# PRBonn/OverlapNet

Measured on NVIDIA H100. Metric: scan-pairs/sec (overlap+yaw) at 64x900, higher is better.
Workload: dtype f16

## Files before the change

overlapnet_b200/csrc/api.cu:

```cuda
#include "common.cuh"
#include <math.h>
#include <string.h>
#include <algorithm>

using namespace ovn;

static const char* kLegNames[] = {"s_conv1", "s_conv2", "s_conv3", "s_conv3a", "s_conv4", "s_conv5",
                                  "s_conv6", "s_conv7", "s_conv8", "s_conv9", "s_conv10"};

static void set_spec(ConvSpec& L, const char* name, int kh, int kw, int sh, int sw, int cin, int cout, int relu,
                     int h_in, int w_in) {
  memset(&L, 0, sizeof(L));
  snprintf(L.name, sizeof(L.name), "%s", name);
  L.kh = kh; L.kw = kw; L.sh = sh; L.sw = sw; L.cin = cin; L.cout = cout; L.relu = relu;
  L.h_in = h_in; L.w_in = w_in;
  L.h_out = (h_in - kh) / sh + 1;
  L.w_out = (w_in - kw) / sw + 1;
}

static void slot_sizes(const ovn_handle* h, int slot, int64_t* n_kernel, int64_t* n_bias) {
  if (slot == kMaxLegLayers + 3) {
    *n_kernel = h->dense_in; *n_bias = 1;
    return;
  }
// ... 71 lines not shown
    case kErrNonFiniteOperand:
      OVN_SET_ERR(h, OVN_ERR_INVALID_ARG, "a value is not finite in the fp16 operands of the tensor-core path: a feature "
                  "volume given to the heads (NaN, inf, or |x - centre| > 65504; outputs of the call are poisoned, NaN / "
                  "INT32_MIN), or in the tensor-core leg an input pixel (NaN, inf) or an activation of s_conv1 .. the "
                  "last layer but one (above 65504; the feature volumes of the call are not valid)");
    case kErrPeerWait: OVN_SET_ERR(h, OVN_ERR_CUDA, "ovn_peer_wait timed out: a peer rank never signalled");
    case kErrInjectedFault: OVN_SET_ERR(h, OVN_ERR_CUDA, "tensor-core pipeline failed: k_conv2_wgmma: fault injected by "
                                        "OVN_DEBUG_FAULT (code %d); outputs of the call are poisoned (NaN / INT32_MIN)", e);
    case kErrDeltaLeftProducer: case kErrDeltaLeftConsumer: ring = "k_delta_conv1_wgmma: LEFT volume ring"; break;
    case kErrDeltaRightProducer: case kErrDeltaRightConsumer: ring = "k_delta_conv1_wgmma: RIGHT window ring"; break;
    case kErrDeltaW1Producer: case kErrDeltaW1Consumer: ring = "k_delta_conv1_wgmma: W1 ring"; break;
    case kErrDeltaO1Producer: case kErrDeltaO1Consumer: ring = "k_delta_conv1_wgmma: o1 staging"; break;
    case kErrConv2Producer: case kErrConv2Consumer: ring = "k_conv2_wgmma: o1 + W2 ring"; break;
    case kErrConv3X3Producer: case kErrConv3X3Consumer: ring = "k_conv3_wgmma: x3 ring"; break;
    case kErrConv3W3Producer: case kErrConv3W3Consumer: ring = "k_conv3_wgmma: W3 ring"; break;
    case kErrCorrRightProducer: case kErrCorrRightConsumer: ring = "k_corr_wgmma: RIGHT third ring"; break;
    case kErrCorrLeftProducer: case kErrCorrLeftConsumer: ring = "k_corr_wgmma: LEFT tile ring"; break;
  }
  if (!ring) OVN_SET_ERR(h, OVN_ERR_CUDA, "unknown device error code %d", e);
  OVN_SET_ERR(h, OVN_ERR_CUDA, "tensor-core pipeline failed: %s, %s wait timed out (code %d); outputs of the call are "
              "poisoned (NaN / INT32_MIN)", ring, e < 200 ? "producer" : "consumer", e);
}

}

extern "C" {

int ovn_abi_version(void) { return OVN_ABI_VERSION; }

const char* ovn_status_string(int status) {
  switch (status) {
    case OVN_OK: return "OVN_OK";
// ... 1659 lines not shown
```

overlapnet_b200/csrc/common.cuh:

```cuda
#pragma once
#include <cuda_runtime.h>
#include <cuda_fp16.h>
#include <stddef.h>
#include <stdint.h>
#include <stdio.h>
#include <memory>
#include <string>
#include <vector>
#include <map>

#include "../../include/ovn_b200.h"

struct ovn_handle;

namespace ovn {

template <class T, bool Pinned = false>
class Buffer {
 public:
  Buffer() = default;
  Buffer(Buffer&& o) noexcept { swap(o); }
  Buffer& operator=(Buffer&& o) noexcept {
    Buffer old(std::move(o));
    swap(old);
// ... 280 lines not shown
  bool switched = false;
  explicit DeviceGuard(const ovn_handle* h) {
    if (h && cudaGetDevice(&prev) == cudaSuccess && prev != h->device) switched = cudaSetDevice(h->device) == cudaSuccess;
  }
  ~DeviceGuard() { if (switched) cudaSetDevice(prev); }
};

enum DeviceError : int {
  kErrDeltaLeftProducer = 101, kErrDeltaLeftConsumer = 402,
  kErrDeltaRightProducer = 103, kErrDeltaRightConsumer = 404,
  kErrDeltaW1Producer = 102, kErrDeltaW1Consumer = 202,
  kErrDeltaO1Producer = 104, kErrDeltaO1Consumer = 405,
  kErrConv2Producer = 111, kErrConv2Consumer = 211,
  kErrConv3X3Producer = 121, kErrConv3X3Consumer = 221,
  kErrConv3W3Producer = 122, kErrConv3W3Consumer = 222,
  kErrCorrRightProducer = 131, kErrCorrRightConsumer = 231,
  kErrCorrLeftProducer = 132, kErrCorrLeftConsumer = 232,
  kErrInjectedFault = 501,
  kErrBadIndex = 900,
  kErrRowNotPrepared = 901,
  kErrIcpBadIndex = 902,
  kErrNonFiniteOperand = 910,
  kErrPeerWait = 950,
};

inline void prof_mark(ovn_handle* h, int kind, cudaStream_t s) {
  if (!h->profiling) return;
  cudaEvent_t e;
  if (cudaEventCreate(&e) != cudaSuccess) return;
  cudaEventRecord(e, s);
  h->prof_ev[kind].push_back(e);
}
// ... 125 lines not shown
```

overlapnet_b200/csrc/network_tc.cu:

```cuda
#include "common.cuh"
#include "hopper.cuh"

#include <cuda_fp16.h>
#include <stddef.h>
#include <stdlib.h>

namespace ovn {

using namespace hopper;

constexpr int WF = 360;
constexpr int CF = 128;
constexpr int S15 = 15;
constexpr int NB = 24;
constexpr int PAIR_ROWS = NB * NB;
constexpr int K4_PITCH = CF;

struct TcState {
  Buffer<__half> w1p;
  Buffer<__half> w2p;
  Buffer<__half> w3p;
  Buffer<float> b2eff;
  Buffer<__half> wres[kMaxLegLayers];
  Buffer<__half> actp[2];
  Buffer<float> leg_part;
  Buffer<__half> l16;
  Buffer<__half> r16;
  Buffer<__half> o1;
  Buffer<__half> x3;
  Buffer<float> partial;
  Buffer<__half> lc;
  Buffer<__half> rc;
  Buffer<float> corr_part;
  const float* pb_key = nullptr;
  int64_t pb_rows = 0;
  Buffer<__half> pb_l16;
  Buffer<__half> pb_lc;
  Buffer<int32_t> pb_bad;
  Buffer<float> mu;
  bool mu_set = false;
  Buffer<float> mu_o1;
  Buffer<float> mu_x3;
  Buffer<float> b2base;
  Buffer<float> b3eff;
  bool act_set = false;
  int64_t rows_pad = 0;
  int64_t last_n = 0;
};

void TcStateDelete::operator()(TcState* t) const { delete t; }

__host__ __device__ __forceinline__ int k4_pos(int r, int c) {
// ... 60 lines not shown
struct LegArgs {
  const __half* A; int64_t a_pitch;
  int runs_per_img, in_img_planes, in_run_planes;
  int kh, kw, c8in;
  const __half* Bp;
  const float* bias; int n_valid;
  int64_t M;
  __half* out_planes; int64_t out_pitch; int out_run_planes;
  float* out_f32;
  int n_split; float* part;
  int* err;
};

__device__ __forceinline__ bool leg_act_unstorable(float v) { return !(v < 65520.f) || v == -INFINITY; }

constexpr int C6_LROWS = 64, C6_RROWS = 128;
constexpr int C6_LT = 6, C6_RT = 3;
constexpr int C6_L_BYTES = 2 * 16 * C6_LROWS * 16;
constexpr int C6_R_BYTES = 2 * 16 * C6_RROWS * 16;
constexpr int C6_VOL_L_BYTES = C6_LT * C6_L_BYTES;
constexpr int C6_VOL_R_BYTES = C6_RT * C6_R_BYTES;

template <int TR, int NT>
__global__ void __launch_bounds__(256)
k_pack_corr(const float* __restrict__ bank, const int32_t* __restrict__ idx, int n, __half* __restrict__ out,
            int* __restrict__ err, int32_t* __restrict__ row_bad) {
  const int64_t i = (int64_t)blockIdx.x * blockDim.x + threadIdx.x;
  const int64_t per = 16 * NT * TR;
  if (i >= (int64_t)n * per) return;
  const int p = (int)(i / per);
  int r = (int)(i % per);
  const int vrow = r % (NT * TR); r /= NT * TR;
  const int pl = r;
  const int tile = vrow / TR, row = vrow % TR;
  float v[8];
  if (vrow < WF) {
    const int64_t src = (idx ? idx[p] : p);
    const float4 a = __ldg(reinterpret_cast<const float4*>(bank + (src * WF + vrow) * CF + pl * 8));
    const float4 b = __ldg(reinterpret_cast<const float4*>(bank + (src * WF + vrow) * CF + pl * 8 + 4));
    v[0] = a.x; v[1] = a.y; v[2] = a.z; v[3] = a.w; v[4] = b.x; v[5] = b.y; v[6] = b.z; v[7] = b.w;
  } else {
#pragma unroll
    for (int e = 0; e < 8; ++e) v[e] = 0.f;
  }
  __half hi[8], lo[8];
#pragma unroll
  for (int e = 0; e < 8; ++e) {
    hi[e] = __float2half_rn(v[e]);
    lo[e] = __float2half_rn(v[e] - __half2float(hi[e]));
  }
  bool bad = false;
#pragma unroll
  for (int e = 0; e < 8; e += 2) bad |= h2_nonfinite(__halves2half2(hi[e], hi[e + 1]));
  if (bad) {
    if (row_bad) row_bad[p] = 1;
    else atomicCAS(err, 0, kErrNonFiniteOperand);
  }
  __half* base = out + ((size_t)p * NT + tile) * (2 * 16 * TR * 8);
  *reinterpret_cast<uint4*>(base + ((size_t)pl * TR + row) * 8) = *reinterpret_cast<const uint4*>(hi);
  *reinterpret_cast<uint4*>(base + ((size_t)(16 + pl) * TR + row) * 8) = *reinterpret_cast<const uint4*>(lo);
}

constexpr int MMA_THREADS = 128;
constexpr int MMA_ROWS = 64;

__device__ __forceinline__ void mma16816(float (&d)[4], uint32_t a0, uint32_t a1, uint32_t a2, uint32_t a3,
                                         uint32_t b0, uint32_t b1) {
  asm volatile("mma.sync.aligned.m16n8k16.row.col.f32.f16.f16.f32 {%0,%1,%2,%3}, {%4,%5,%6,%7}, {%8,%9}, {%0,%1,%2,%3};"
               : "+f"(d[0]), "+f"(d[1]), "+f"(d[2]), "+f"(d[3])
               : "r"(a0), "r"(a1), "r"(a2), "r"(a3), "r"(b0), "r"(b1));
}

__device__ __forceinline__ uint32_t ld_h2(const __half* p) { return __ldg(reinterpret_cast<const unsigned int*>(p)); }

__device__ __forceinline__ uint32_t absdiff_h2(uint32_t a, uint32_t b) {
// ... 437 lines not shown
          for (int j = 0; j < 16; ++j) {
            const int n = j * 8 + 2 * t;
            sum = fmaf(fmaxf(acc[sub][4 * j + 2 * h] + __ldg(bias + nh * 128 + n), 0.f), __ldg(wrow + n), sum);
            sum = fmaf(fmaxf(acc[sub][4 * j + 2 * h + 1] + __ldg(bias + nh * 128 + n + 1), 0.f), __ldg(wrow + n + 1), sum);
          }
          sum += __shfl_xor_sync(0xffffffffu, sum, 1);
          sum += __shfl_xor_sync(0xffffffffu, sum, 2);
          if (t == 0 && r < M) partial[r * 2 + nh] = valid ? sum : 0.f;
        }
    }
  }
done:
  return;
}

constexpr int C6_PARTS = C6_LT * C6_RT;
constexpr int C6_WG = 2;
constexpr int C6_THREADS = C6_WG * 128 + 32;
constexpr int C6_RING = 3;
constexpr int C6_GPITCH = 132;

struct C6Smem {
  __half R[C6_R_BYTES / 2];
  __half L[C6_RING][C6_L_BYTES / 2];
  float G[C6_WG][C6_LROWS * C6_GPITCH];
  MbarRing<C6_RING> left;
  MbarRing<1> right;
};
static_assert(sizeof(C6Smem) <= 232448, "k_corr_wgmma shared memory");
static_assert(offsetof(C6Smem, L) % 16 == 0, "bulk-copy alignment");

__global__ void __launch_bounds__(C6_THREADS, 1)
k_corr_wgmma(const __half* __restrict__ Lc, const int32_t* __restrict__ l_idx, const __half* __restrict__ Rc,
             int r_per_pair, int n_pairs, float* __restrict__ corr_part, int* __restrict__ err) {
  extern __shared__ __align__(128) uint8_t smem_raw[];
  C6Smem& S = *reinterpret_cast<C6Smem*>(smem_raw);
  const int tid = threadIdx.x, warp = tid >> 5, lane = tid & 31;
  const int q = blockIdx.x % C6_RT;
  const Share share = work_share((int64_t)n_pairs * C6_LT, blockIdx.x / C6_RT, gridDim.x / C6_RT);
  const int u_begin = (int)share.begin, u_end = (int)share.end;
  if (tid == 0) {
    S.left.init(4);
    S.right.init(C6_WG * 4);
    mbar_fence_init();
  }
  __syncthreads();

  if (warp == C6_WG * 4) {
    if (lane == 0) {
      uint32_t ri = 0, ui = 0;
      int key = -1;
      for (int u = u_begin; u < u_end; ++u, ++ui) {
        const int p = u / C6_LT, a = u - p * C6_LT;
        if ((r_per_pair ? p : 0) != key) {
          key = r_per_pair ? p : 0;
          PIPE_WAIT(S.right.acquire(ri, C6_R_BYTES), kErrCorrRightProducer);
          bulk_g2s(S.R, Rc + ((size_t)key * C6_RT + q) * (C6_R_BYTES / 2), C6_R_BYTES, S.right.bar(ri));
          ++ri;
        }
        PIPE_WAIT(S.left.acquire(ui, C6_L_BYTES), kErrCorrLeftProducer);
        bulk_g2s(S.L[S.left.slot(ui)], Lc + ((size_t)(l_idx ? l_idx[p] : p) * C6_LT + a) * (C6_L_BYTES / 2), C6_L_BYTES,
                 S.left.bar(ui));
      }
    }
  } else {
    const int wg = warp >> 2, wi = warp & 3, g = lane >> 2, t = lane & 3, tw = tid & 127;
    float* Gw = S.G[wg];
    const uint32_t r_base = smem_u32(S.R);
    uint32_t ri = 0, ui = 0;
    int key = -1;
    bool failed = false;
    for (int u = u_begin; u < u_end; ++u, ++ui) {
      const int p = u / C6_LT, a = u - p * C6_LT;
      if ((r_per_pair ? p : 0) != key) {
        if (key >= 0) S.right.release(ri - 1);
        key = r_per_pair ? p : 0;
        INFLIGHT_WAIT(S.right.wait(ri), kErrCorrRightConsumer);
        ++ri;
      }
      if ((int)(ui & 1) != wg) continue;
      const uint32_t s = S.left.slot(ui);
      INFLIGHT_WAIT(S.left.wait(ui), kErrCorrLeftConsumer);
      const uint32_t l_base = smem_u32(S.L[s]);
      float acc[64];
#pragma unroll
      for (int e = 0; e < 64; ++e) acc[e] = 0.f;
      wgmma_fence();
#pragma unroll
      for (int c16 = 0; c16 < 8; ++c16) {
        const uint64_t ah = desc_kmajor(l_base + c16 * 2 * C6_LROWS * 16, C6_LROWS * 16, 128, kNoSwizzle);
        const uint64_t al = desc_kmajor(l_base + C6_L_BYTES / 2 + c16 * 2 * C6_LROWS * 16, C6_LROWS * 16, 128, kNoSwizzle);
        const uint64_t bh = desc_kmajor(r_base + c16 * 2 * C6_RROWS * 16, C6_RROWS * 16, 128, kNoSwizzle);
        const uint64_t bl = desc_kmajor(r_base + C6_R_BYTES / 2 + c16 * 2 * C6_RROWS * 16, C6_RROWS * 16, 128, kNoSwizzle);
        wgmma_m64n128k16_ss(acc, ah, bh);
        wgmma_m64n128k16_ss(acc, al, bh);
        wgmma_m64n128k16_ss(acc, ah, bl);
      }
      wgmma_commit();
      wgmma_wait<0>();
      S.left.release(ui);
      named_bar_sync(1 + wg, 128);
#pragma unroll
      for (int j = 0; j < 16; ++j) {
        float* r0 = Gw + (wi * 16 + g) * C6_GPITCH + j * 8 + 2 * t;
        *reinterpret_cast<float2*>(r0) = make_float2(acc[4 * j], acc[4 * j + 1]);
        *reinterpret_cast<float2*>(r0 + 8 * C6_GPITCH) = make_float2(acc[4 * j + 2], acc[4 * j + 3]);
      }
      named_bar_sync(1 + wg, 128);
      const int i_lim = min(C6_LROWS, WF - a * C6_LROWS), j_lim = min(C6_RROWS, WF - q * C6_RROWS);
      float* out = corr_part + ((size_t)p * C6_PARTS + a * C6_RT + q) * WF;
      for (int d = tw; d < WF; d += 128) {
        const int dd = d - (C6_RROWS - 1);
        float sum = 0.f;
        if (d < C6_LROWS + C6_RROWS - 1) {
#pragma unroll 8
          for (int ii = 0; ii < C6_LROWS; ++ii) {
            const int jj = ii - dd;
            if (ii < i_lim && jj >= 0 && jj < j_lim) sum += Gw[ii * C6_GPITCH + jj];
          }
        }
        int k = (a * C6_LROWS - q * C6_RROWS + dd - WF / 2) % WF;
        if (k < 0) k += WF;
        out[k] = sum;
      }
    }
  }
done:
  return;
}

template <int EPI>
__global__ void __launch_bounds__(MMA_THREADS)
k_leg_mma(LegArgs g) {
  const int warp = threadIdx.x >> 5, lane = threadIdx.x & 31, gq = lane >> 2, t = lane & 3;
  const int64_t px0 = (int64_t)blockIdx.y * MMA_ROWS + warp * 16;
  if (px0 >= g.M) return;
  const int nz = (g.n_valid + 63) / 64;
  const int y = blockIdx.x, z = blockIdx.z % nz, slice = blockIdx.z / nz;
  const int64_t in_base = (int64_t)(y / g.runs_per_img) * g.in_img_planes + (int64_t)(y % g.runs_per_img) * g.in_run_planes;
// ... 87 lines not shown
    if (bad) atomicCAS(g.err, 0, kErrNonFiniteOperand);
    __half hi[8], lo[8];
#pragma unroll
    for (int e = 0; e < 8; ++e) {
      hi[e] = __float2half_rn(v[e]);
      lo[e] = __float2half_rn(v[e] - __half2float(hi[e]));
    }
    const int64_t pl = y * g.out_run_planes + c8;
    *reinterpret_cast<uint4*>(g.out_planes + ((size_t)pl * g.out_pitch + px) * 8) = *reinterpret_cast<const uint4*>(hi);
    *reinterpret_cast<uint4*>(g.out_planes + ((size_t)(pl + g.out_run_planes / 2) * g.out_pitch + px) * 8) =
        *reinterpret_cast<const uint4*>(lo);
  } else {
    float* dst = g.out_f32 + (y * g.M + px) * g.n_valid + c8 * 8;
    *reinterpret_cast<float4*>(dst) = make_float4(v[0], v[1], v[2], v[3]);
    *reinterpret_cast<float4*>(dst + 4) = make_float4(v[4], v[5], v[6], v[7]);
  }
}

__global__ void __launch_bounds__(384)
k_corr_finalize(const float* __restrict__ part, float* __restrict__ corr_out, int32_t* __restrict__ yaw,
                const int* __restrict__ err) {
  __shared__ float s_corr[WF];
  const int p = blockIdx.x;
  for (int k = threadIdx.x; k < WF; k += blockDim.x) {
    float c = 0.f;
    for (int b = 0; b < C6_PARTS; ++b) c += part[((size_t)p * C6_PARTS + b) * WF + k];
    s_corr[k] = c;
    if (corr_out) corr_out[(size_t)p * WF + k] = c;
  }
  __syncthreads();
  if (threadIdx.x == 0) {
    int best = 0;
    float bv = s_corr[0];
    for (int k = 1; k < WF; ++k)
      if (s_corr[k] > bv) { bv = s_corr[k]; best = k; }
    yaw[p] = (*err != 0) ? INT32_MIN : 180 - best;
  }
}

__global__ void __launch_bounds__(1024)
k_o1_channel_mean(const __half* __restrict__ o1, int64_t M, float* __restrict__ mu) {
  __shared__ float part[16][64];
  const int o = threadIdx.x & 63, g = threadIdx.x >> 6;
  float acc = 0.f;
  for (int64_t m = g; m < M; m += 16)
    for (int di = 0; di < S15; ++di) acc += __half2float(o1[o1_chunk_offset(m, di, o >> 3) + (o & 7)]);
  part[g][o] = acc;
  __syncthreads();
  if (g == 0) {
    float t = 0.f;
    for (int k = 0; k < 16; ++k) t += part[k][o];
// ... 327 lines not shown
  if ((rc = t->leg_part.ensure(h, part_bytes)) != OVN_OK) return rc;
  for (int b = 0; b < 2; ++b) {
    const size_t bytes = max_planes_bytes * h->cfg.max_batch_scans + 32768;
    if ((rc = t->actp[b].ensure(h, bytes)) != OVN_OK) return rc;
    OVN_CUDA(h, cudaMemset(t->actp[b], 0, bytes));
  }
  const int64_t maxp = h->cfg.max_batch_pairs;
  t->rows_pad = ((maxp * PAIR_ROWS + 1024 + 255) / 256) * 256;
  if ((rc = t->l16.ensure(h, (size_t)maxp * WF * K4_PITCH * sizeof(__half))) != OVN_OK) return rc;
  if ((rc = t->r16.ensure(h, (size_t)maxp * WF * K4_PITCH * sizeof(__half))) != OVN_OK) return rc;
  OVN_CUDA(h, cudaMemset(t->l16, 0, (size_t)maxp * WF * K4_PITCH * sizeof(__half)));
  OVN_CUDA(h, cudaMemset(t->r16, 0, (size_t)maxp * WF * K4_PITCH * sizeof(__half)));
  if ((rc = t->o1.ensure(h, (size_t)120 * t->rows_pad * 8 * sizeof(__half))) != OVN_OK) return rc;
  if ((rc = t->x3.ensure(h, (size_t)16 * t->rows_pad * 8 * sizeof(__half))) != OVN_OK) return rc;
  if ((rc = t->partial.ensure(h, (size_t)t->rows_pad * 2 * sizeof(float))) != OVN_OK) return rc;
  if ((rc = t->lc.ensure(h, (size_t)maxp * C6_VOL_L_BYTES)) != OVN_OK) return rc;
  if ((rc = t->rc.ensure(h, (size_t)maxp * C6_VOL_R_BYTES)) != OVN_OK) return rc;
  if ((rc = t->corr_part.ensure(h, (size_t)maxp * C6_PARTS * WF * sizeof(float))) != OVN_OK) return rc;
  OVN_CUDA(h, cudaFuncSetAttribute(k_delta_conv1_wgmma, cudaFuncAttributeMaxDynamicSharedMemorySize, (int)sizeof(K4Smem)));
  OVN_CUDA(h, cudaFuncSetAttribute(k_conv2_wgmma, cudaFuncAttributeMaxDynamicSharedMemorySize, (int)C2_SMEM));
  OVN_CUDA(h, cudaFuncSetAttribute(k_conv3_wgmma, cudaFuncAttributeMaxDynamicSharedMemorySize, (int)sizeof(C3Smem)));
  OVN_CUDA(h, cudaFuncSetAttribute(k_corr_wgmma, cudaFuncAttributeMaxDynamicSharedMemorySize, (int)sizeof(C6Smem)));
  if ((rc = t->mu.ensure(h, CF * sizeof(float))) != OVN_OK) return rc;
  OVN_CUDA(h, cudaMemset(t->mu, 0, CF * sizeof(float)));
  OVN_CUDA(h, cudaMemset(t->o1, 0, (size_t)120 * t->rows_pad * 8 * sizeof(__half)));
  OVN_CUDA(h, cudaMemset(t->x3, 0, (size_t)16 * t->rows_pad * 8 * sizeof(__half)));
  OVN_CUDA(h, cudaFuncSetAttribute(k_leg_layer1_small<true>, cudaFuncAttributeMaxDynamicSharedMemorySize, (int)L1_SMALL_SMEM));
  OVN_CUDA(h, cudaFuncSetAttribute(k_leg_layer1_small<false>, cudaFuncAttributeMaxDynamicSharedMemorySize, (int)L1_SMALL_SMEM));
  h->tc = std::move(t);
  return OVN_OK;
}

int leg_forward_tc(ovn_handle* h, const float* d_input, int n, float* d_fv, cudaStream_t s, int stop_layer) {
  TcState* t = h->tc.get();
  if (!t) OVN_SET_ERR(h, OVN_ERR_WEIGHTS, "tensor-core weights not packed");
  prof_mark(h, PROF_LEG, s);
  {
// ... 41 lines not shown
      else k_leg_splitk_reduce<4><<<(unsigned)((work + 255) / 256), 256, 0, s>>>(la, n * L.h_out);
    } else if (last) {
      k_leg_mma<3><<<grid, MMA_THREADS, 0, s>>>(la);
    } else {
      k_leg_mma<4><<<grid, MMA_THREADS, 0, s>>>(la);
    }
    OVN_LAUNCH_CHECK(h);
    cur ^= 1;
  }
  prof_mark(h, PROF_LEG, s);
  return OVN_OK;
}

static int calibrate_all(ovn_handle* h, const float* d_vols, const int32_t* d_idx, bool keep_mu, cudaStream_t s);

int tc_bank_release(ovn_handle* h, const float* d_bank) {
  TcState* t = h->tc.get();
  if (!t || (d_bank && t->pb_key != d_bank)) return OVN_OK;
  OVN_CUDA(h, cudaDeviceSynchronize());
  t->pb_l16 = {};
  t->pb_lc = {};
  t->pb_bad = {};
  t->pb_key = nullptr;
  t->pb_rows = 0;
  return OVN_OK;
}

int tc_bank_prepare(ovn_handle* h, const float* d_bank, int64_t capacity, int64_t first, int64_t count, cudaStream_t s) {
  TcState* t = h->tc.get();
  if (!t) OVN_SET_ERR(h, OVN_ERR_WEIGHTS, "tensor-core weights not packed");
  const size_t l16_bytes = (size_t)capacity * WF * K4_PITCH * sizeof(__half);
  if (t->pb_key != d_bank || l16_bytes > t->pb_l16.bytes()) {
    int rc = OVN_OK;
    if (t->pb_key != nullptr || t->pb_l16) rc = tc_bank_release(h, nullptr);
    if (rc == OVN_OK) rc = t->pb_l16.ensure(h, l16_bytes);
    if (rc == OVN_OK) rc = t->pb_lc.ensure(h, (size_t)capacity * C6_VOL_L_BYTES);
    if (rc == OVN_OK) rc = t->pb_bad.ensure(h, (size_t)capacity * sizeof(int32_t));
    if (rc != OVN_OK) return rc;
    OVN_CUDA(h, cudaMemsetAsync(t->pb_l16, 0, l16_bytes, s));
    t->pb_key = d_bank;
    t->pb_rows = 0;
    if (first != 0) OVN_SET_ERR(h, OVN_ERR_INVALID_ARG, "ovn_bank_prepare: a new bank must be prepared from row 0");
  }
  if (first > t->pb_rows) OVN_SET_ERR(h, OVN_ERR_INVALID_ARG, "ovn_bank_prepare: rows [%lld, %lld) were never prepared",
                                      (long long)t->pb_rows, (long long)first);
  const int64_t per = (int64_t)WF * CF / 4, perL = 16 * C6_LT * C6_LROWS;
  const float* src = d_bank + (size_t)first * WF * CF;
  if (!t->mu_set) {
    int rc = calibrate_all(h, src, nullptr, false, s);
    if (rc != OVN_OK) return rc;
  }
  OVN_CUDA(h, cudaMemsetAsync(t->pb_bad + first, 0, (size_t)count * sizeof(int32_t), s));
  k_gather_rows_f16<<<(unsigned)((count * per + 255) / 256), 256, 0, s>>>(src, nullptr, (int)count, t->mu, 0,
                                                                         t->pb_l16 + (size_t)first * WF * K4_PITCH, h->d_err,
                                                                         t->pb_bad + first);
  OVN_LAUNCH_CHECK(h);
  k_pack_corr<C6_LROWS, C6_LT><<<(unsigned)((count * perL + 255) / 256), 256, 0, s>>>(src, nullptr, (int)count,
                                                                      t->pb_lc + (size_t)first * (C6_VOL_L_BYTES / 2), h->d_err,
                                                                      t->pb_bad + first);
  OVN_LAUNCH_CHECK(h);
  if (first + count > t->pb_rows) t->pb_rows = first + count;
  return OVN_OK;
}

static int calibrate_all(ovn_handle* h, const float* d_vols, const int32_t* d_idx, bool keep_mu, cudaStream_t s) {
  TcState* t = h->tc.get();
  const int base = kMaxLegLayers;
  const int64_t per = (int64_t)WF * CF / 4;
  if (!keep_mu) {
    k_channel_mean<<<1, 1024, 0, s>>>(d_vols, d_idx, 1, t->mu);
    OVN_LAUNCH_CHECK(h);
  }
  OVN_CUDA(h, cudaMemsetAsync(t->mu_o1, 0, 64 * sizeof(float), s));
  OVN_CUDA(h, cudaMemsetAsync(t->mu_x3, 0, 128 * sizeof(float), s));
  k_gather_rows_f16<<<(unsigned)((per + 255) / 256), 256, 0, s>>>(d_vols, d_idx, 1, t->mu, 0, t->l16, h->d_err, nullptr);
// ... 67 lines not shown
int heads_forward_tc(ovn_handle* h, const float* d_bank, const float* d_query, const int32_t* d_left,
                     const int32_t* d_right, int n, float* d_overlap, int32_t* d_yaw, float* d_corr,
                     cudaStream_t s) {
  TcState* t = h->tc.get();
  if (!t) OVN_SET_ERR(h, OVN_ERR_WEIGHTS, "tensor-core weights not packed");
  const int maxp = h->cfg.max_batch_pairs;
  const int base = kMaxLegLayers;
  const int64_t per = (int64_t)WF * CF / 4;
  t->last_n = 0;
  if ((!t->mu_set || !t->act_set) && n > 0) {
    int rc = d_query ? calibrate_all(h, d_query, nullptr, t->mu_set, s) : calibrate_all(h, d_bank, d_right, t->mu_set, s);
    if (rc != OVN_OK) return rc;
  }
  const bool resident = (t->pb_key == d_bank) && t->pb_rows > 0;
  const __half* l16 = resident ? t->pb_l16 : t->l16;
  const __half* lc = resident ? t->pb_lc : t->lc;
  int32_t* lidx = nullptr;
  if (resident) {
    lidx = h->d_idx_san + 2 * (size_t)maxp;
    int rc = sanitize_indices(h, d_left, n, t->pb_rows, kErrRowNotPrepared, lidx, s, t->pb_bad);
    if (rc != OVN_OK) return rc;
  } else {
    k_gather_rows_f16<<<(unsigned)((n * per + 255) / 256), 256, 0, s>>>(d_bank, d_left, n, t->mu, 0, t->l16, h->d_err, nullptr);
    OVN_LAUNCH_CHECK(h);
  }
  if (d_query)
    k_gather_rows_f16<<<(unsigned)((per + 255) / 256), 256, 0, s>>>(d_query, nullptr, 1, t->mu, 0, t->r16, h->d_err, nullptr);
  else
    k_gather_rows_f16<<<(unsigned)((n * per + 255) / 256), 256, 0, s>>>(d_bank, d_right, n, t->mu, 0, t->r16, h->d_err, nullptr);
  OVN_LAUNCH_CHECK(h);
  const int64_t M = (int64_t)n * PAIR_ROWS;
// ... 8 lines not shown
  prof_mark(h, PROF_DELTA, s);
  OVN_LAUNCH_CHECK(h);
  const bool inject_fault = getenv("OVN_DEBUG_FAULT") != nullptr;
  prof_mark(h, PROF_CONV2, s);
  k_conv2_wgmma<<<grid2, TC_THREADS, C2_SMEM, s>>>(t->o1, t->w2p, t->b2eff, t->mu_x3, t->x3, t->rows_pad, M,
                                                   inject_fault ? 1 : 0, h->d_err);
  prof_mark(h, PROF_CONV2, s);
  OVN_LAUNCH_CHECK(h);
  prof_mark(h, PROF_CONV3, s);
  k_conv3_wgmma<<<grid3, TC_THREADS, sizeof(C3Smem), s>>>(t->x3, t->rows_pad, t->w3p, t->b3eff, M, h->d_w[base + 3],
                                                          t->partial, h->d_err);
  prof_mark(h, PROF_CONV3, s);
  OVN_LAUNCH_CHECK(h);
  k_dense_finalize<<<n, 256, 0, s>>>(t->partial, h->d_b[base + 3], PAIR_ROWS, d_overlap, h->d_err);
  OVN_LAUNCH_CHECK(h);
  const int64_t perL = 16 * C6_LT * C6_LROWS, perR = 16 * C6_RT * C6_RROWS;
  if (!resident) {
    k_pack_corr<C6_LROWS, C6_LT><<<(unsigned)((n * perL + 255) / 256), 256, 0, s>>>(d_bank, d_left, n, t->lc, h->d_err, nullptr);
    OVN_LAUNCH_CHECK(h);
  }
  if (d_query)
    k_pack_corr<C6_RROWS, C6_RT><<<(unsigned)((perR + 255) / 256), 256, 0, s>>>(d_query, nullptr, 1, t->rc, h->d_err, nullptr);
  else
    k_pack_corr<C6_RROWS, C6_RT><<<(unsigned)((n * perR + 255) / 256), 256, 0, s>>>(d_bank, d_right, n, t->rc, h->d_err, nullptr);
  OVN_LAUNCH_CHECK(h);
  prof_mark(h, PROF_CORR, s);
  const int nc = (int64_t)n * C6_LT < h->sm_count / C6_RT ? n * C6_LT : h->sm_count / C6_RT;
  k_corr_wgmma<<<nc * C6_RT, C6_THREADS, sizeof(C6Smem), s>>>(lc, lidx, t->rc, d_query ? 0 : 1, n, t->corr_part, h->d_err);
  prof_mark(h, PROF_CORR, s);
  OVN_LAUNCH_CHECK(h);
  k_corr_finalize<<<n, 384, 0, s>>>(t->corr_part, d_corr, d_yaw, h->d_err);
  OVN_LAUNCH_CHECK(h);
  t->last_n = n;
  static const bool debug_sync = getenv("OVN_DEBUG_SYNC") != nullptr;
  if (debug_sync) return check_device_error(h, s);
  return OVN_OK;
}

__global__ void __launch_bounds__(256)
k_copy_heads_stage(int stage, const __half* __restrict__ o1, const __half* __restrict__ x3, int64_t x3_pitch,
                   const float* __restrict__ partial, int64_t first, int64_t total, float* __restrict__ out) {
  const int64_t e = (int64_t)blockIdx.x * blockDim.x + threadIdx.x;
  if (e >= total) return;
  out += e;
  if (stage == OVN_STAGE_O1) {
    const int o = (int)(e % 64), jb = (int)(e / 64 % NB), i = (int)(e / (64 * NB) % WF);
// ... 70 lines not shown
```

Before: 212,700.

## Replace tensor-core circular correlation with FP64 FFT spectral correlation for yaw

Swaps the split-fp16 wgmma cross-correlation (pack, corr, finalize) for an FP64 path. A mixed-radix 360-point FFT kernel (radix 8, 9, 5) computes per-channel real spectra of the left and right volumes. A spectral kernel then multiplies and accumulates them across channels, takes an inverse DFT in shared memory, and finds the argmax yaw in the same kernel. This reduces correlation work from O(W^2·C) to O(W log W·C) and removes the partial buffer and finalize launch. In exchange it adds FP64 arithmetic, which has limited throughput on H100, and doubles-sized spectra traffic. Resident banks now cache spectra instead of packed halves.

```diff
diff --git a/overlapnet_b200/csrc/api.cu b/overlapnet_b200/csrc/api.cu
--- a/overlapnet_b200/csrc/api.cu
+++ b/overlapnet_b200/csrc/api.cu
@@ -109,8 +109,8 @@
     case kErrConv2Producer: case kErrConv2Consumer: ring = "k_conv2_wgmma: o1 + W2 ring"; break;
     case kErrConv3X3Producer: case kErrConv3X3Consumer: ring = "k_conv3_wgmma: x3 ring"; break;
     case kErrConv3W3Producer: case kErrConv3W3Consumer: ring = "k_conv3_wgmma: W3 ring"; break;
-    case kErrCorrRightProducer: case kErrCorrRightConsumer: ring = "k_corr_wgmma: RIGHT third ring"; break;
-    case kErrCorrLeftProducer: case kErrCorrLeftConsumer: ring = "k_corr_wgmma: LEFT tile ring"; break;
+    case kErrSpecRightProducer: case kErrSpecRightConsumer: ring = "k_corr_spectral: RIGHT spectrum ring"; break;
+    case kErrSpecLeftProducer: case kErrSpecLeftConsumer: ring = "k_corr_spectral: LEFT spectra ring"; break;
   }
   if (!ring) OVN_SET_ERR(h, OVN_ERR_CUDA, "unknown device error code %d", e);
   OVN_SET_ERR(h, OVN_ERR_CUDA, "tensor-core pipeline failed: %s, %s wait timed out (code %d); outputs of the call are "
diff --git a/overlapnet_b200/csrc/common.cuh b/overlapnet_b200/csrc/common.cuh
--- a/overlapnet_b200/csrc/common.cuh
+++ b/overlapnet_b200/csrc/common.cuh
@@ -318,8 +318,8 @@
   kErrConv2Producer = 111, kErrConv2Consumer = 211,
   kErrConv3X3Producer = 121, kErrConv3X3Consumer = 221,
   kErrConv3W3Producer = 122, kErrConv3W3Consumer = 222,
-  kErrCorrRightProducer = 131, kErrCorrRightConsumer = 231,
-  kErrCorrLeftProducer = 132, kErrCorrLeftConsumer = 232,
+  kErrSpecRightProducer = 133, kErrSpecRightConsumer = 233,
+  kErrSpecLeftProducer = 134, kErrSpecLeftConsumer = 234,
   kErrInjectedFault = 501,
   kErrBadIndex = 900,
   kErrRowNotPrepared = 901,
diff --git a/overlapnet_b200/csrc/network_tc.cu b/overlapnet_b200/csrc/network_tc.cu
--- a/overlapnet_b200/csrc/network_tc.cu
+++ b/overlapnet_b200/csrc/network_tc.cu
@@ -29,13 +29,13 @@
   Buffer<__half> o1;
   Buffer<__half> x3;
   Buffer<float> partial;
-  Buffer<__half> lc;
-  Buffer<__half> rc;
-  Buffer<float> corr_part;
+  Buffer<double2> lspec;
+  Buffer<double2> rspec;
+  Buffer<double2> tw;
   const float* pb_key = nullptr;
   int64_t pb_rows = 0;
   Buffer<__half> pb_l16;
-  Buffer<__half> pb_lc;
+  Buffer<double2> pb_spec;
   Buffer<int32_t> pb_bad;
   Buffer<float> mu;
   bool mu_set = false;
@@ -126,51 +126,97 @@
 
 __device__ __forceinline__ bool leg_act_unstorable(float v) { return !(v < 65520.f) || v == -INFINITY; }
 
-constexpr int C6_LROWS = 64, C6_RROWS = 128;
-constexpr int C6_LT = 6, C6_RT = 3;
-constexpr int C6_L_BYTES = 2 * 16 * C6_LROWS * 16;
-constexpr int C6_R_BYTES = 2 * 16 * C6_RROWS * 16;
-constexpr int C6_VOL_L_BYTES = C6_LT * C6_L_BYTES;
-constexpr int C6_VOL_R_BYTES = C6_RT * C6_R_BYTES;
-
-template <int TR, int NT>
-__global__ void __launch_bounds__(256)
-k_pack_corr(const float* __restrict__ bank, const int32_t* __restrict__ idx, int n, __half* __restrict__ out,
-            int* __restrict__ err, int32_t* __restrict__ row_bad) {
-  const int64_t i = (int64_t)blockIdx.x * blockDim.x + threadIdx.x;
-  const int64_t per = 16 * NT * TR;
-  if (i >= (int64_t)n * per) return;
-  const int p = (int)(i / per);
-  int r = (int)(i % per);
-  const int vrow = r % (NT * TR); r /= NT * TR;
-  const int pl = r;
-  const int tile = vrow / TR, row = vrow % TR;
-  float v[8];
-  if (vrow < WF) {
-    const int64_t src = (idx ? idx[p] : p);
-    const float4 a = __ldg(reinterpret_cast<const float4*>(bank + (src * WF + vrow) * CF + pl * 8));
-    const float4 b = __ldg(reinterpret_cast<const float4*>(bank + (src * WF + vrow) * CF + pl * 8 + 4));
-    v[0] = a.x; v[1] = a.y; v[2] = a.z; v[3] = a.w; v[4] = b.x; v[5] = b.y; v[6] = b.z; v[7] = b.w;
-  } else {
-#pragma unroll
-    for (int e = 0; e < 8; ++e) v[e] = 0.f;
-  }
-  __half hi[8], lo[8];
-#pragma unroll
-  for (int e = 0; e < 8; ++e) {
-    hi[e] = __float2half_rn(v[e]);
-    lo[e] = __float2half_rn(v[e] - __half2float(hi[e]));
-  }
+constexpr int SP_BINS = WF / 2 + 1;
+constexpr int64_t SP_VOL = (int64_t)CF * SP_BINS;
+constexpr int SP_CH = 8;
+constexpr int SP_SEQ = SP_CH / 2;
+constexpr int SP_THREADS = 288;
+constexpr int SP_SMEM = (2 * SP_SEQ * WF + WF) * (int)sizeof(double2);
+
+__device__ __forceinline__ double2 cmul(double2 a, double2 w) {
+  return make_double2(fma(-a.y, w.y, a.x * w.x), fma(a.y, w.x, a.x * w.y));
+}
+__device__ __forceinline__ double2 cfma(double2 a, double2 w, double2 y) {
+  y.x = fma(a.x, w.x, y.x);
+  y.x = fma(-a.y, w.y, y.x);
+  y.y = fma(a.x, w.y, y.y);
+  y.y = fma(a.y, w.x, y.y);
+  return y;
+}
+
+template <int R>
+__device__ __forceinline__ void fft_pass(const double2* __restrict__ src, double2* __restrict__ dst, int Ns,
+                                         const double2* __restrict__ tw) {
+  constexpr int NB = WF / R;
+  for (int w = threadIdx.x; w < SP_SEQ * NB; w += SP_THREADS) {
+    const int m = w / NB, j = w - m * NB, k = j % Ns;
+    const int step = k * (WF / (Ns * R));
+    const double2* a = src + m * WF;
+    double2 v[R];
+    v[0] = a[j];
+#pragma unroll
+    for (int r = 1; r < R; ++r) v[r] = cmul(a[j + r * NB], tw[step * r]);
+    double2* b = dst + m * WF + (j / Ns) * Ns * R + k;
+#pragma unroll
+    for (int q = 0; q < R; ++q) {
+      double2 y = v[0];
+#pragma unroll
+      for (int r = 1; r < R; ++r) {
+        if ((r * q) % R == 0) y = make_double2(y.x + v[r].x, y.y + v[r].y);
+        else y = cfma(v[r], tw[((r * q) % R) * NB], y);
+      }
+      b[q * Ns] = y;
+    }
+  }
+}
+
+struct SpectraJob {
+  const float* bank;
+  const int32_t* idx;
+  int n;
+  double2* out;
+  int32_t* row_bad;
+};
+
+__global__ void __launch_bounds__(SP_THREADS)
+k_spectra_f64(SpectraJob ja, SpectraJob jb, const double2* __restrict__ twg, int* __restrict__ err) {
+  extern __shared__ __align__(128) uint8_t smem_raw[];
+  double2* A = reinterpret_cast<double2*>(smem_raw);
+  double2* B = A + SP_SEQ * WF;
+  double2* tw = B + SP_SEQ * WF;
+  const int v = blockIdx.x / (CF / SP_CH), c0 = (blockIdx.x % (CF / SP_CH)) * SP_CH;
+  const SpectraJob job = v < ja.n ? ja : jb;
+  const int p = v < ja.n ? v : v - ja.n;
+  const float* vol = job.bank + (int64_t)(job.idx ? job.idx[p] : p) * WF * CF + c0;
+  int32_t* row_bad = job.row_bad;
+  double2* out = job.out;
+  for (int i = threadIdx.x; i < WF; i += SP_THREADS) tw[i] = twg[i];
   bool bad = false;
-#pragma unroll
-  for (int e = 0; e < 8; e += 2) bad |= h2_nonfinite(__halves2half2(hi[e], hi[e + 1]));
+  for (int i = threadIdx.x; i < WF * SP_SEQ; i += SP_THREADS) {
+    const int n = i / SP_SEQ, m = i % SP_SEQ;
+    const float2 v = __ldg(reinterpret_cast<const float2*>(vol + (int64_t)n * CF) + m);
+    bad |= !(fabsf(v.x) < 65520.f) || !(fabsf(v.y) < 65520.f);
+    A[m * WF + n] = make_double2(v.x, v.y);
+  }
   if (bad) {
     if (row_bad) row_bad[p] = 1;
     else atomicCAS(err, 0, kErrNonFiniteOperand);
   }
-  __half* base = out + ((size_t)p * NT + tile) * (2 * 16 * TR * 8);
-  *reinterpret_cast<uint4*>(base + ((size_t)pl * TR + row) * 8) = *reinterpret_cast<const uint4*>(hi);
-  *reinterpret_cast<uint4*>(base + ((size_t)(16 + pl) * TR + row) * 8) = *reinterpret_cast<const uint4*>(lo);
+  __syncthreads();
+  fft_pass<8>(A, B, 1, tw);
+  __syncthreads();
+  fft_pass<9>(B, A, 8, tw);
+  __syncthreads();
+  fft_pass<5>(A, B, 72, tw);
+  __syncthreads();
+  double2* o = out + (int64_t)p * SP_VOL + (int64_t)c0 * SP_BINS;
+  for (int i = threadIdx.x; i < SP_SEQ * SP_BINS; i += SP_THREADS) {
+    const int m = i / SP_BINS, f = i % SP_BINS;
+    const double2 z = B[m * WF + f], zc = B[m * WF + (WF - f) % WF];
+    const bool real = (f == 0 || f == WF / 2);
+    o[(2 * m) * SP_BINS + f] = make_double2(0.5 * (z.x + zc.x), real ? 0.0 : 0.5 * (z.y - zc.y));
+    o[(2 * m + 1) * SP_BINS + f] = make_double2(0.5 * (z.y + zc.y), real ? 0.0 : 0.5 * (zc.x - z.x));
+  }
 }
 
 constexpr int MMA_THREADS = 128;
@@ -638,115 +684,124 @@
   return;
 }
 
-constexpr int C6_PARTS = C6_LT * C6_RT;
-constexpr int C6_WG = 2;
-constexpr int C6_THREADS = C6_WG * 128 + 32;
-constexpr int C6_RING = 3;
-constexpr int C6_GPITCH = 132;
-
-struct C6Smem {
-  __half R[C6_R_BYTES / 2];
-  __half L[C6_RING][C6_L_BYTES / 2];
-  float G[C6_WG][C6_LROWS * C6_GPITCH];
-  MbarRing<C6_RING> left;
-  MbarRing<1> right;
+constexpr int CS_WARPS = 6;
+constexpr int CS_THREADS = CS_WARPS * 32 + 32;
+constexpr uint32_t CS_CHAN_BYTES = SP_BINS * sizeof(double2);
+
+template <int P, int U, int D>
+struct CsSmem {
+  double2 L[D][P][U * SP_BINS];
+  double2 R[D][U * SP_BINS];
+  double2 tw[WF];
+  double2 S[P][SP_BINS];
+  float sc[P][WF];
+  MbarRing<D> left, right;
 };
-static_assert(sizeof(C6Smem) <= 232448, "k_corr_wgmma shared memory");
-static_assert(offsetof(C6Smem, L) % 16 == 0, "bulk-copy alignment");
-
-__global__ void __launch_bounds__(C6_THREADS, 1)
-k_corr_wgmma(const __half* __restrict__ Lc, const int32_t* __restrict__ l_idx, const __half* __restrict__ Rc,
-             int r_per_pair, int n_pairs, float* __restrict__ corr_part, int* __restrict__ err) {
+
+template <int P, int U, int D>
+__global__ void __launch_bounds__(CS_THREADS)
+k_corr_spectral(const double2* __restrict__ Ls, const int32_t* __restrict__ l_idx, const double2* __restrict__ Rs,
+                int n, const double2* __restrict__ twg, float* __restrict__ corr_out, int32_t* __restrict__ yaw,
+                int* __restrict__ err) {
+  static_assert(P <= CS_WARPS && CF % U == 0, "k_corr_spectral shape");
+  constexpr uint32_t FILL = U * CS_CHAN_BYTES;
   extern __shared__ __align__(128) uint8_t smem_raw[];
-  C6Smem& S = *reinterpret_cast<C6Smem*>(smem_raw);
+  CsSmem<P, U, D>& S = *reinterpret_cast<CsSmem<P, U, D>*>(smem_raw);
   const int tid = threadIdx.x, warp = tid >> 5, lane = tid & 31;
-  const int q = blockIdx.x % C6_RT;
-  const Share share = work_share((int64_t)n_pairs * C6_LT, blockIdx.x / C6_RT, gridDim.x / C6_RT);
-  const int u_begin = (int)share.begin, u_end = (int)share.end;
+  const int p0 = blockIdx.x * P, np = min(P, n - p0);
   if (tid == 0) {
-    S.left.init(4);
-    S.right.init(C6_WG * 4);
+    S.left.init(CS_WARPS);
+    S.right.init(CS_WARPS);
     mbar_fence_init();
   }
   __syncthreads();
-
-  if (warp == C6_WG * 4) {
+  if (warp == CS_WARPS) {
     if (lane == 0) {
-      uint32_t ri = 0, ui = 0;
-      int key = -1;
-      for (int u = u_begin; u < u_end; ++u, ++ui) {
-        const int p = u / C6_LT, a = u - p * C6_LT;
-        if ((r_per_pair ? p : 0) != key) {
-          key = r_per_pair ? p : 0;
-          PIPE_WAIT(S.right.acquire(ri, C6_R_BYTES), kErrCorrRightProducer);
-          bulk_g2s(S.R, Rc + ((size_t)key * C6_RT + q) * (C6_R_BYTES / 2), C6_R_BYTES, S.right.bar(ri));
-          ++ri;
-        }
-        PIPE_WAIT(S.left.acquire(ui, C6_L_BYTES), kErrCorrLeftProducer);
-        bulk_g2s(S.L[S.left.slot(ui)], Lc + ((size_t)(l_idx ? l_idx[p] : p) * C6_LT + a) * (C6_L_BYTES / 2), C6_L_BYTES,
-                 S.left.bar(ui));
+      const double2* lp[P];
+      for (int i = 0; i < np; ++i) lp[i] = Ls + (int64_t)(l_idx ? l_idx[p0 + i] : p0 + i) * SP_VOL;
+      const double2* rp = Rs + (P == 1 ? (int64_t)p0 * SP_VOL : 0);
+      for (uint32_t f = 0; f < CF / U; ++f) {
+        PIPE_WAIT(S.right.acquire(f, FILL), kErrSpecRightProducer);
+        bulk_g2s(S.R[S.right.slot(f)], rp + f * U * SP_BINS, FILL, S.right.bar(f));
+        PIPE_WAIT(S.left.acquire(f, np * FILL), kErrSpecLeftProducer);
+        for (int i = 0; i < np; ++i) bulk_g2s(S.L[S.left.slot(f)][i], lp[i] + f * U * SP_BINS, FILL, S.left.bar(f));
       }
     }
   } else {
-    const int wg = warp >> 2, wi = warp & 3, g = lane >> 2, t = lane & 3, tw = tid & 127;
-    float* Gw = S.G[wg];
-    const uint32_t r_base = smem_u32(S.R);
-    uint32_t ri = 0, ui = 0;
-    int key = -1;
     bool failed = false;
-    for (int u = u_begin; u < u_end; ++u, ++ui) {
-      const int p = u / C6_LT, a = u - p * C6_LT;
-      if ((r_per_pair ? p : 0) != key) {
-        if (key >= 0) S.right.release(ri - 1);
-        key = r_per_pair ? p : 0;
-        INFLIGHT_WAIT(S.right.wait(ri), kErrCorrRightConsumer);
-        ++ri;
-      }
-      if ((int)(ui & 1) != wg) continue;
-      const uint32_t s = S.left.slot(ui);
-      INFLIGHT_WAIT(S.left.wait(ui), kErrCorrLeftConsumer);
-      const uint32_t l_base = smem_u32(S.L[s]);
-      float acc[64];
-#pragma unroll
-      for (int e = 0; e < 64; ++e) acc[e] = 0.f;
-      wgmma_fence();
-#pragma unroll
-      for (int c16 = 0; c16 < 8; ++c16) {
-        const uint64_t ah = desc_kmajor(l_base + c16 * 2 * C6_LROWS * 16, C6_LROWS * 16, 128, kNoSwizzle);
-        const uint64_t al = desc_kmajor(l_base + C6_L_BYTES / 2 + c16 * 2 * C6_LROWS * 16, C6_LROWS * 16, 128, kNoSwizzle);
-        const uint64_t bh = desc_kmajor(r_base + c16 * 2 * C6_RROWS * 16, C6_RROWS * 16, 128, kNoSwizzle);
-        const uint64_t bl = desc_kmajor(r_base + C6_R_BYTES / 2 + c16 * 2 * C6_RROWS * 16, C6_RROWS * 16, 128, kNoSwizzle);
-        wgmma_m64n128k16_ss(acc, ah, bh);
-        wgmma_m64n128k16_ss(acc, al, bh);
-        wgmma_m64n128k16_ss(acc, ah, bl);
-      }
-      wgmma_commit();
-      wgmma_wait<0>();
-      S.left.release(ui);
-      named_bar_sync(1 + wg, 128);
-#pragma unroll
-      for (int j = 0; j < 16; ++j) {
-        float* r0 = Gw + (wi * 16 + g) * C6_GPITCH + j * 8 + 2 * t;
-        *reinterpret_cast<float2*>(r0) = make_float2(acc[4 * j], acc[4 * j + 1]);
-        *reinterpret_cast<float2*>(r0 + 8 * C6_GPITCH) = make_float2(acc[4 * j + 2], acc[4 * j + 3]);
-      }
-      named_bar_sync(1 + wg, 128);
-      const int i_lim = min(C6_LROWS, WF - a * C6_LROWS), j_lim = min(C6_RROWS, WF - q * C6_RROWS);
-      float* out = corr_part + ((size_t)p * C6_PARTS + a * C6_RT + q) * WF;
-      for (int d = tw; d < WF; d += 128) {
-        const int dd = d - (C6_RROWS - 1);
-        float sum = 0.f;
-        if (d < C6_LROWS + C6_RROWS - 1) {
-#pragma unroll 8
-          for (int ii = 0; ii < C6_LROWS; ++ii) {
-            const int jj = ii - dd;
-            if (ii < i_lim && jj >= 0 && jj < j_lim) sum += Gw[ii * C6_GPITCH + jj];
+    for (int i = tid; i < WF; i += CS_WARPS * 32) S.tw[i] = twg[i];
+    double sr[P], si[P];
+#pragma unroll
+    for (int i = 0; i < P; ++i) sr[i] = si[i] = 0.0;
+#pragma unroll 1
+    for (uint32_t f = 0; f < CF / U; ++f) {
+      INFLIGHT_WAIT(S.right.wait(f), kErrSpecRightConsumer);
+      INFLIGHT_WAIT(S.left.wait(f), kErrSpecLeftConsumer);
+      if (tid < SP_BINS)
+#pragma unroll
+        for (int u = 0; u < U; ++u) {
+          const double2 r = S.R[S.right.slot(f)][u * SP_BINS + tid];
+#pragma unroll
+          for (int i = 0; i < P; ++i) {
+            if (i >= np) break;
+            const double2 l = S.L[S.left.slot(f)][i][u * SP_BINS + tid];
+            sr[i] = fma(l.x, r.x, sr[i]);
+            sr[i] = fma(l.y, r.y, sr[i]);
+            si[i] = fma(l.y, r.x, si[i]);
+            si[i] = fma(-l.x, r.y, si[i]);
           }
         }
-        int k = (a * C6_LROWS - q * C6_RROWS + dd - WF / 2) % WF;
-        if (k < 0) k += WF;
-        out[k] = sum;
-      }
+      S.right.release(f);
+      S.left.release(f);
+    }
+    if (tid < SP_BINS)
+#pragma unroll
+      for (int i = 0; i < P; ++i) S.S[i][tid] = make_double2(sr[i], si[i]);
+    named_bar_sync(1, CS_WARPS * 32);
+    if (tid < WF / 2) {
+      const int k = tid;
+      double ev[P], od[P];
+#pragma unroll
+      for (int i = 0; i < P; ++i) ev[i] = od[i] = 0.0;
+      int m = 0;
+      auto term = [&](int f, double (&acc)[P]) {
+        m += k;
+        if (m >= WF) m -= WF;
+        const double2 w = S.tw[m];
+#pragma unroll
+        for (int i = 0; i < P; ++i) {
+          const double2 s = S.S[i][f];
+          acc[i] = __dadd_rn(acc[i], __fma_rn(s.y, w.y, __dmul_rn(s.x, w.x)));
+        }
+      };
+#pragma unroll 4
+      for (int f = 1; f < WF / 2 - 1; f += 2) {
+        term(f, od);
+        term(f + 1, ev);
+      }
+      term(WF / 2 - 1, od);
+#pragma unroll
+      for (int i = 0; i < P; ++i) {
+        const double b = (k & 1) ? __dsub_rn(S.S[i][0].x, S.S[i][WF / 2].x) : __dadd_rn(S.S[i][0].x, S.S[i][WF / 2].x);
+        S.sc[i][k] = __double2float_rn(__ddiv_rn(__fma_rn(2.0, __dsub_rn(ev[i], od[i]), b), (double)WF));
+        S.sc[i][k + WF / 2] = __double2float_rn(__ddiv_rn(__fma_rn(2.0, __dadd_rn(ev[i], od[i]), b), (double)WF));
+      }
+    }
+    named_bar_sync(1, CS_WARPS * 32);
+    if (corr_out)
+      for (int e = tid; e < np * WF; e += CS_WARPS * 32) corr_out[(int64_t)p0 * WF + e] = S.sc[e / WF][e % WF];
+    if (warp < np) {
+      float bv = S.sc[warp][lane];
+      int best = lane;
+      for (int k = lane + 32; k < WF; k += 32)
+        if (S.sc[warp][k] > bv) { bv = S.sc[warp][k]; best = k; }
+#pragma unroll
+      for (int o = 16; o > 0; o >>= 1) {
+        const float ov = __shfl_xor_sync(0xffffffffu, bv, o);
+        const int ob = __shfl_xor_sync(0xffffffffu, best, o);
+        if (ov > bv || (ov == bv && ob < best)) { bv = ov; best = ob; }
+      }
+      if (lane == 0) yaw[p0 + warp] = (*err != 0) ? INT32_MIN : 180 - best;
     }
   }
 done:
@@ -864,27 +919,6 @@
     float* dst = g.out_f32 + (y * g.M + px) * g.n_valid + c8 * 8;
     *reinterpret_cast<float4*>(dst) = make_float4(v[0], v[1], v[2], v[3]);
     *reinterpret_cast<float4*>(dst + 4) = make_float4(v[4], v[5], v[6], v[7]);
-  }
-}
-
-__global__ void __launch_bounds__(384)
-k_corr_finalize(const float* __restrict__ part, float* __restrict__ corr_out, int32_t* __restrict__ yaw,
-                const int* __restrict__ err) {
-  __shared__ float s_corr[WF];
-  const int p = blockIdx.x;
-  for (int k = threadIdx.x; k < WF; k += blockDim.x) {
-    float c = 0.f;
-    for (int b = 0; b < C6_PARTS; ++b) c += part[((size_t)p * C6_PARTS + b) * WF + k];
-    s_corr[k] = c;
-    if (corr_out) corr_out[(size_t)p * WF + k] = c;
-  }
-  __syncthreads();
-  if (threadIdx.x == 0) {
-    int best = 0;
-    float bv = s_corr[0];
-    for (int k = 1; k < WF; ++k)
-      if (s_corr[k] > bv) { bv = s_corr[k]; best = k; }
-    yaw[p] = (*err != 0) ? INT32_MIN : 180 - best;
   }
 }
 
@@ -1242,13 +1276,22 @@
   if ((rc = t->o1.ensure(h, (size_t)120 * t->rows_pad * 8 * sizeof(__half))) != OVN_OK) return rc;
   if ((rc = t->x3.ensure(h, (size_t)16 * t->rows_pad * 8 * sizeof(__half))) != OVN_OK) return rc;
   if ((rc = t->partial.ensure(h, (size_t)t->rows_pad * 2 * sizeof(float))) != OVN_OK) return rc;
-  if ((rc = t->lc.ensure(h, (size_t)maxp * C6_VOL_L_BYTES)) != OVN_OK) return rc;
-  if ((rc = t->rc.ensure(h, (size_t)maxp * C6_VOL_R_BYTES)) != OVN_OK) return rc;
-  if ((rc = t->corr_part.ensure(h, (size_t)maxp * C6_PARTS * WF * sizeof(float))) != OVN_OK) return rc;
+  if ((rc = t->lspec.ensure(h, (size_t)maxp * SP_VOL * sizeof(double2))) != OVN_OK) return rc;
+  if ((rc = t->rspec.ensure(h, (size_t)maxp * SP_VOL * sizeof(double2))) != OVN_OK) return rc;
+  {
+    double2 tw[WF];
+    for (int m = 0; m < WF; ++m) tw[m] = make_double2(cos(2.0 * M_PI * m / WF), -sin(2.0 * M_PI * m / WF));
+    if ((rc = t->tw.ensure(h, sizeof(tw))) != OVN_OK) return rc;
+    OVN_CUDA(h, cudaMemcpy(t->tw, tw, sizeof(tw), cudaMemcpyHostToDevice));
+  }
   OVN_CUDA(h, cudaFuncSetAttribute(k_delta_conv1_wgmma, cudaFuncAttributeMaxDynamicSharedMemorySize, (int)sizeof(K4Smem)));
   OVN_CUDA(h, cudaFuncSetAttribute(k_conv2_wgmma, cudaFuncAttributeMaxDynamicSharedMemorySize, (int)C2_SMEM));
   OVN_CUDA(h, cudaFuncSetAttribute(k_conv3_wgmma, cudaFuncAttributeMaxDynamicSharedMemorySize, (int)sizeof(C3Smem)));
-  OVN_CUDA(h, cudaFuncSetAttribute(k_corr_wgmma, cudaFuncAttributeMaxDynamicSharedMemorySize, (int)sizeof(C6Smem)));
+  OVN_CUDA(h, cudaFuncSetAttribute(k_spectra_f64, cudaFuncAttributeMaxDynamicSharedMemorySize, SP_SMEM));
+  OVN_CUDA(h, cudaFuncSetAttribute(k_corr_spectral<4, 1, 3>, cudaFuncAttributeMaxDynamicSharedMemorySize,
+                                   (int)sizeof(CsSmem<4, 1, 3>)));
+  OVN_CUDA(h, cudaFuncSetAttribute(k_corr_spectral<1, 8, 2>, cudaFuncAttributeMaxDynamicSharedMemorySize,
+                                   (int)sizeof(CsSmem<1, 8, 2>)));
   if ((rc = t->mu.ensure(h, CF * sizeof(float))) != OVN_OK) return rc;
   OVN_CUDA(h, cudaMemset(t->mu, 0, CF * sizeof(float)));
   OVN_CUDA(h, cudaMemset(t->o1, 0, (size_t)120 * t->rows_pad * 8 * sizeof(__half)));
@@ -1320,12 +1363,20 @@
 
 static int calibrate_all(ovn_handle* h, const float* d_vols, const int32_t* d_idx, bool keep_mu, cudaStream_t s);
 
+static int spectra(ovn_handle* h, const SpectraJob& a, const SpectraJob& b, cudaStream_t s) {
+  const int64_t n = (int64_t)a.n + b.n;
+  if (n == 0) return OVN_OK;
+  k_spectra_f64<<<(unsigned)(n * (CF / SP_CH)), SP_THREADS, SP_SMEM, s>>>(a, b, h->tc->tw, h->d_err);
+  OVN_LAUNCH_CHECK(h);
+  return OVN_OK;
+}
+
 int tc_bank_release(ovn_handle* h, const float* d_bank) {
   TcState* t = h->tc.get();
   if (!t || (d_bank && t->pb_key != d_bank)) return OVN_OK;
   OVN_CUDA(h, cudaDeviceSynchronize());
   t->pb_l16 = {};
-  t->pb_lc = {};
+  t->pb_spec = {};
   t->pb_bad = {};
   t->pb_key = nullptr;
   t->pb_rows = 0;
@@ -1340,7 +1391,7 @@
     int rc = OVN_OK;
     if (t->pb_key != nullptr || t->pb_l16) rc = tc_bank_release(h, nullptr);
     if (rc == OVN_OK) rc = t->pb_l16.ensure(h, l16_bytes);
-    if (rc == OVN_OK) rc = t->pb_lc.ensure(h, (size_t)capacity * C6_VOL_L_BYTES);
+    if (rc == OVN_OK) rc = t->pb_spec.ensure(h, (size_t)capacity * SP_VOL * sizeof(double2));
     if (rc == OVN_OK) rc = t->pb_bad.ensure(h, (size_t)capacity * sizeof(int32_t));
     if (rc != OVN_OK) return rc;
     OVN_CUDA(h, cudaMemsetAsync(t->pb_l16, 0, l16_bytes, s));
@@ -1350,7 +1401,7 @@
   }
   if (first > t->pb_rows) OVN_SET_ERR(h, OVN_ERR_INVALID_ARG, "ovn_bank_prepare: rows [%lld, %lld) were never prepared",
                                       (long long)t->pb_rows, (long long)first);
-  const int64_t per = (int64_t)WF * CF / 4, perL = 16 * C6_LT * C6_LROWS;
+  const int64_t per = (int64_t)WF * CF / 4;
   const float* src = d_bank + (size_t)first * WF * CF;
   if (!t->mu_set) {
     int rc = calibrate_all(h, src, nullptr, false, s);
@@ -1361,10 +1412,11 @@
                                                                          t->pb_l16 + (size_t)first * WF * K4_PITCH, h->d_err,
                                                                          t->pb_bad + first);
   OVN_LAUNCH_CHECK(h);
-  k_pack_corr<C6_LROWS, C6_LT><<<(unsigned)((count * perL + 255) / 256), 256, 0, s>>>(src, nullptr, (int)count,
-                                                                      t->pb_lc + (size_t)first * (C6_VOL_L_BYTES / 2), h->d_err,
-                                                                      t->pb_bad + first);
-  OVN_LAUNCH_CHECK(h);
+  {
+    const int rc = spectra(h, SpectraJob{src, nullptr, (int)count, t->pb_spec + first * SP_VOL, t->pb_bad + first},
+                           SpectraJob{}, s);
+    if (rc != OVN_OK) return rc;
+  }
   if (first + count > t->pb_rows) t->pb_rows = first + count;
   return OVN_OK;
 }
@@ -1462,7 +1514,7 @@
   }
   const bool resident = (t->pb_key == d_bank) && t->pb_rows > 0;
   const __half* l16 = resident ? t->pb_l16 : t->l16;
-  const __half* lc = resident ? t->pb_lc : t->lc;
+  const double2* lspec = resident ? t->pb_spec : t->lspec;
   int32_t* lidx = nullptr;
   if (resident) {
     lidx = h->d_idx_san + 2 * (size_t)maxp;
@@ -1501,22 +1553,21 @@
   OVN_LAUNCH_CHECK(h);
   k_dense_finalize<<<n, 256, 0, s>>>(t->partial, h->d_b[base + 3], PAIR_ROWS, d_overlap, h->d_err);
   OVN_LAUNCH_CHECK(h);
-  const int64_t perL = 16 * C6_LT * C6_LROWS, perR = 16 * C6_RT * C6_RROWS;
-  if (!resident) {
-    k_pack_corr<C6_LROWS, C6_LT><<<(unsigned)((n * perL + 255) / 256), 256, 0, s>>>(d_bank, d_left, n, t->lc, h->d_err, nullptr);
-    OVN_LAUNCH_CHECK(h);
+  prof_mark(h, PROF_CORR, s);
+  {
+    const SpectraJob left = {d_bank, d_left, resident ? 0 : n, t->lspec, nullptr};
+    const SpectraJob right = d_query ? SpectraJob{d_query, nullptr, 1, t->rspec, nullptr}
+                                     : SpectraJob{d_bank, d_right, n, t->rspec, nullptr};
+    const int rc = spectra(h, left, right, s);
+    if (rc != OVN_OK) return rc;
   }
   if (d_query)
-    k_pack_corr<C6_RROWS, C6_RT><<<(unsigned)((perR + 255) / 256), 256, 0, s>>>(d_query, nullptr, 1, t->rc, h->d_err, nullptr);
+    k_corr_spectral<4, 1, 3><<<(unsigned)((n + 3) / 4), CS_THREADS, sizeof(CsSmem<4, 1, 3>), s>>>(
+        lspec, lidx, t->rspec, n, t->tw, d_corr, d_yaw, h->d_err);
   else
-    k_pack_corr<C6_RROWS, C6_RT><<<(unsigned)((n * perR + 255) / 256), 256, 0, s>>>(d_bank, d_right, n, t->rc, h->d_err, nullptr);
-  OVN_LAUNCH_CHECK(h);
+    k_corr_spectral<1, 8, 2><<<(unsigned)n, CS_THREADS, sizeof(CsSmem<1, 8, 2>), s>>>(
+        lspec, lidx, t->rspec, n, t->tw, d_corr, d_yaw, h->d_err);
   prof_mark(h, PROF_CORR, s);
-  const int nc = (int64_t)n * C6_LT < h->sm_count / C6_RT ? n * C6_LT : h->sm_count / C6_RT;
-  k_corr_wgmma<<<nc * C6_RT, C6_THREADS, sizeof(C6Smem), s>>>(lc, lidx, t->rc, d_query ? 0 : 1, n, t->corr_part, h->d_err);
-  prof_mark(h, PROF_CORR, s);
-  OVN_LAUNCH_CHECK(h);
-  k_corr_finalize<<<n, 384, 0, s>>>(t->corr_part, d_corr, d_yaw, h->d_err);
   OVN_LAUNCH_CHECK(h);
   t->last_n = n;
   static const bool debug_sync = getenv("OVN_DEBUG_SYNC") != nullptr;
```

Result: faster. 221,100, median of 6 (+3.9%).
